# NOAA-GFDL/icebergs

Hardware: AMD Instinct MI355X
Metric: berg_steps_per_sec (higher is better)
Workload: dtype f64; 1 GPU; BASELINE configs[4] per-GPU share with configs[1] physics: 10000000 synthetic bergs/GPU (random mass classes), 360x200 lat-lon ocean grid, RK4 drag+Coriolis+melt+mass spreading, dt=1800 s, ignore_traj=T; bergs_per_gpu=10000000, grid=360x200, exchange=none (1 GPU), bergs_alive_at_end=9999583

## Files before the change

icebergs_amd/csrc/kid_berg_kernel.hpp:

```cpp
#pragma once
#include "kid_device.hpp"
#include "kid_thermo.hpp"
#include "kid_footloose.hpp"
#include "kid_launch_select.hpp"

namespace {
using namespace kid;

struct BergPtrs {
  double *f[KID_NB_F64];
  int32_t *i[KID_NB_I32];
  int64_t *id;
  const double *orient;
};
struct Flags { int has_static, has_fl, store_env, footprint, no_diag; };
typedef __attribute__((address_space(1))) double gdouble;
typedef __attribute__((address_space(1))) int32_t gint32;
typedef __attribute__((address_space(1))) char gchar;
__device__ __forceinline__ double ldg(const double *q, long long k) { return *(const gdouble *)((const gchar *)q + (size_t)((unsigned)k << 3)); }
__device__ __forceinline__ int32_t ldg(const int32_t *q, long long k) { return *(const gint32 *)((const gchar *)q + (size_t)((unsigned)k << 2)); }
__device__ __forceinline__ void keep(double x) { asm volatile("" ::"v"(x)); }
__device__ __forceinline__ void keep(int32_t x) { asm volatile("" ::"v"(x)); }
__device__ __forceinline__ void stg(double *q, long long k, double v) { *(gdouble *)((gchar *)q + (size_t)((unsigned)k << 3)) = v; }
__device__ __forceinline__ void stg(int32_t *q, long long k, int32_t v) { *(gint32 *)((gchar *)q + (size_t)((unsigned)k << 2)) = v; }
template <int K> struct Fl {
#define KID_X(name, k1, k2, k3) static __device__ __forceinline__ int name(const Flags &f) { if constexpr (K == 1) return k1; else if constexpr (K == 2) return k2; else if constexpr (K == 3) return k3; else return f.name; }
  KID_X(has_static, 0, 0, 0) KID_X(has_fl, 0, 1, 0) KID_X(store_env, 0, f.store_env, 1) KID_X(footprint, 0, 0, 0) KID_X(no_diag, 0, 0, 0)
#undef KID_X
};

#ifndef KID_WAVES_PER_EU
#define KID_WAVES_PER_EU 2
#endif
#ifndef KID_HOT_WG
#define KID_HOT_WG 64
#endif
#ifdef KID_EXP_NO_PRIO
#define KID_PRIO_ON false
#else
#define KID_PRIO_ON true
#endif
#ifndef KID_GENERAL_WAVES_PER_EU
#define KID_GENERAL_WAVES_PER_EU 2
#endif
struct StageTab { double *val; int32_t *key; unsigned long long *mask; long long cap; };
enum { KID_RB_NX8 = 10, KID_RB_NX4 = 4 };
struct RebinTab { BergPtrs dst; const void *xs[KID_RB_NX8 + KID_RB_NX4]; void *xd[KID_RB_NX8 + KID_RB_NX4]; int n8, n4; unsigned long long moved, surplus; };
struct Redo { int *list; int *count; long long k0, klen; int *lane; int step;
              int *fl_cursor; int32_t *fl_counter; long long fl_capacity; int fl_iNg; unsigned fl_step;
              StageTab st{};
              const RebinTab *rb = nullptr; const unsigned *perm = nullptr; };
constexpr unsigned long long rb_bit(int f) { return 1ull << f; }
constexpr unsigned long long KID_RB_DYN = rb_bit(KID_B_LON) | rb_bit(KID_B_LAT) | rb_bit(KID_B_UVEL) | rb_bit(KID_B_VVEL) | rb_bit(KID_B_AXN) | rb_bit(KID_B_AYN) |
                                          rb_bit(KID_B_BXN) | rb_bit(KID_B_BYN) | rb_bit(KID_B_XI) | rb_bit(KID_B_YJ);
constexpr unsigned long long KID_RB_ENV = rb_bit(KID_B_UO) | rb_bit(KID_B_VO) | rb_bit(KID_B_UI) | rb_bit(KID_B_VI) | rb_bit(KID_B_UA) | rb_bit(KID_B_VA) |
                                          rb_bit(KID_B_SSH_X) | rb_bit(KID_B_SSH_Y) | rb_bit(KID_B_SST) | rb_bit(KID_B_SSS) | rb_bit(KID_B_CN) | rb_bit(KID_B_HI);
constexpr unsigned long long rb_thermo_fields(int K) {
  return rb_bit(KID_B_MASS) | rb_bit(KID_B_THICKNESS) | rb_bit(KID_B_WIDTH) | rb_bit(KID_B_LENGTH) | rb_bit(KID_B_MASS_OF_BITS) | (K == 3 ? KID_RB_ENV : 0ull);
}
static_assert(KID_NB_F64 <= 64, "one bit per fp64 field");
typedef const __attribute__((address_space(4))) RebinTab cRebinTab;
template <bool REBIN> struct DstTab { static __device__ __forceinline__ const BergPtrs &get(const BergPtrs &b, const Redo &) { return b; } };
template <> struct DstTab<true> { static __device__ __forceinline__ const auto &get(const BergPtrs &, const Redo &r) { return ((cRebinTab *)r.rb)->dst; } };
template <class BD> __device__ __forceinline__ void rebin_copy_row(const BergPtrs &b, const BD &bd, const unsigned *perm, unsigned long long m, bool cell, long long k) {
  const long long ks = (long long)perm[k];
  int32_t ci = 0, cj = 0;
  if (cell) { ci = ldg(b.i[KID_BI_INE], ks); cj = ldg(b.i[KID_BI_JNE], ks); }
  while (m != 0ull) {
    int f[8];
    double v[8];
#pragma unroll
    for (int q = 0; q < 8; ++q) { f[q] = (m != 0ull) ? (int)__ffsll((long long)m) - 1 : -1; m &= m - 1ull; }
#pragma unroll
    for (int q = 0; q < 8; ++q) v[q] = (f[q] >= 0) ? ldg(b.f[f[q]], ks) : 0.;
#pragma unroll
    for (int q = 0; q < 8; ++q) if (f[q] >= 0) stg(bd.f[f[q]], k, v[q]);
  }
  if (cell) { stg(bd.i[KID_BI_INE], k, ci); stg(bd.i[KID_BI_JNE], k, cj); }
}
#ifdef KID_EXP_NUM_VGPR
#define KID_NUM_VGPR_ATTR __attribute__((amdgpu_num_vgpr(KID_EXP_NUM_VGPR)))
#else
#define KID_NUM_VGPR_ATTR
#endif
#ifndef KID_FLP_SLOTS
#define KID_FLP_SLOTS KID_MAXRUN
#define KID_FLP_CHUNK 10
#endif
#ifndef KID_HOT3_SLOTS
#define KID_HOT3_SLOTS 11
#define KID_HOT3_CHUNK 11
#endif
template <bool RK, bool OLD_ORDER, unsigned PH, bool FAST, int K> struct HotCfg {
#if defined(KID_EXACT_MATH) || defined(KID_EXP_NO_HOT3)
  static constexpr bool three = false;
#else
  static constexpr bool three = FAST && RK && OLD_ORDER && (K == 1 || K == 3) && (PH & PH_EVOLVE) != 0 && KID_HOT_WG == 64;
#endif
  static constexpr int slots = three ? KID_HOT3_SLOTS : ((FAST && K == 2) ? KID_FLP_SLOTS : KID_MAXRUN);
  static constexpr int chunk = three ? KID_HOT3_CHUNK : ((FAST && K == 2) ? KID_FLP_CHUNK : KID_CHUNK);
  static constexpr int waves = !FAST ? KID_GENERAL_WAVES_PER_EU : (three ? 3 : KID_WAVES_PER_EU);
};
template <bool S> __device__ __forceinline__ auto &scatter_of(Seg &seg, StageSeg &sseg) { if constexpr (S) return sseg; else return seg; }
template <bool RK, bool OLD_ORDER, unsigned PH, bool FAST, int K = 0, bool STAGE = false, bool REBIN = false>
__global__ void KID_NUM_VGPR_ATTR __launch_bounds__(FAST ? KID_HOT_WG : 256, (HotCfg<RK, OLD_ORDER, PH, FAST, K>::waves)) berg_kernel(const DevGrid *__restrict__ gtab, const kid_params *__restrict__ pp, const BergPtrs *__restrict__ bt, const long long n,
                                                   double *__restrict__ acc, const size_t ncell, const Flags fl, const Redo redo) {
  static_assert(!REBIN || (FAST && RK && OLD_ORDER && !STAGE && (K == 1 || K == 3) && PH == (PH_EVOLVE | PH_THERMO | PH_SPREAD)), "the re-binning instance is a plain hot build");
  const kid_params &p = *pp;
  const BergPtrs &b = *bt;
  const auto &bd = DstTab<REBIN>::get(b, redo);
  const DevGrid &g = *gtab;
  constexpr bool SCATTER = (PH & (PH_THERMO | PH_SPREAD)) != 0;
  constexpr int WG_WAVES = FAST ? KID_HOT_WG / 64 : 4;
  using Cfg = HotCfg<RK, OLD_ORDER, PH, FAST, K>;
  constexpr int SLOTS = Cfg::slots, CHUNK = Cfg::chunk;
  __shared__ double lds_vals[SCATTER ? seg_lds_doubles(WG_WAVES, CHUNK) : 1];
  __shared__ int lds_ints[seg_lds_ints(WG_WAVES, CHUNK)];
  __shared__ __attribute__((aligned(16))) double lds_pk[FAST ? WG_WAVES * SLOTS * PK_STRIDE : 2];
  const long long total = FAST ? redo.klen : (long long)(*redo.count);
  const long long bdim = FAST ? (long long)KID_HOT_WG : (long long)blockDim.x;
  long long tid = (long long)blockIdx.x * bdim + threadIdx.x;
  for (bool first = true; FAST ? first : (tid - threadIdx.x < total); first = false, tid += (long long)gridDim.x * bdim) {
  KID_TICK(-1);
  if (FAST && KID_PRIO_ON) __builtin_amdgcn_s_setprio(3);
  const bool inrange = tid < total;
  const long long k = inrange ? (FAST ? redo.k0 + tid : (long long)redo.list[tid]) : 0ll;
  const long long kk = inrange ? k : (n - 1);
  if constexpr (STAGE) { if (inrange) redo.st.key[k] = -1; }
  long long ks = kk;
  [[maybe_unused]] double x8[KID_RB_NX8];
  [[maybe_unused]] int32_t x4[KID_RB_NX4];
  if constexpr (REBIN) {
    ks = (long long)redo.perm[kk];
    cRebinTab &rb = *(cRebinTab *)redo.rb;
#pragma unroll
    for (int q = 0; q < KID_RB_NX8; ++q) x8[q] = (q < rb.n8) ? ldg((const double *)rb.xs[q], ks) : 0.;
#pragma unroll
    for (int q = 0; q < KID_RB_NX4; ++q) x4[q] = (q < rb.n4) ? ldg((const int32_t *)rb.xs[KID_RB_NX8 + q], ks) : 0;
  }
  const int32_t alive_v = ldg(b.i[KID_BI_ALIVE], ks);
  const int32_t lane_v = FAST ? ldg(redo.lane ? (const int32_t *)redo.lane : (const int32_t *)b.i[KID_BI_ALIVE], ks) : 0;
  BergDyn d;
  d.ine = ldg(b.i[KID_BI_INE], ks); d.jne = ldg(b.i[KID_BI_JNE], ks);
  d.xi = ldg(b.f[KID_B_XI], ks); d.yj = ldg(b.f[KID_B_YJ], ks);
  d.lon = ldg(b.f[KID_B_LON], ks); d.lat = ldg(b.f[KID_B_LAT], ks);
  d.uvel = ldg(b.f[KID_B_UVEL], ks); d.vvel = ldg(b.f[KID_B_VVEL], ks);
  d.uvel_prev = 0.; d.vvel_prev = 0.;
  d.axn = 0.; d.ayn = 0.; d.bxn = 0.; d.byn = 0.;
  if (PH & PH_EVOLVE) {
    d.axn = ldg(b.f[KID_B_AXN], ks); d.ayn = ldg(b.f[KID_B_AYN], ks);
    if (!RK) { d.bxn = ldg(b.f[KID_B_BXN], ks); d.byn = ldg(b.f[KID_B_BYN], ks); }
  }
  BergThermo t;
  t.M = ldg(b.f[KID_B_MASS], ks); t.T = ldg(b.f[KID_B_THICKNESS], ks); t.W = ldg(b.f[KID_B_WIDTH], ks); t.L = ldg(b.f[KID_B_LENGTH], ks);
  t.n_bonds = Sw<K>::iceberg_bonds_on(p) ? ldg(b.i[KID_BI_N_BONDS], ks) : 0;
  t.static_berg = Fl<K>::has_static(fl) ? ldg(b.f[KID_B_STATIC_BERG], ks) : 0.;
  const bool halo = Fl<K>::has_static(fl) ? (ldg(b.f[KID_B_HALO_BERG], ks) >= 0.5) : false;
  constexpr bool SCATTER_ = (PH & (PH_THERMO | PH_SPREAD)) != 0;
  constexpr bool PARK = FAST && SCATTER_ && (PH & PH_EVOLVE) != 0;
  constexpr bool LATE_PARK = PARK && (PH & PH_FL) != 0;
  static_assert(!REBIN || PARK, "the re-binning instance reads its row at the head of the kernel only (ks); the loads further down use kk");
  double park_ms = 0., park_bits = 0., park_hd = 0., park_flk = 0., park_flbits = 0., park_flbergy = 0.;
  if constexpr (PARK) {
    park_ms = ldg(b.f[KID_B_MASS_SCALING], ks); park_bits = ldg(b.f[KID_B_MASS_OF_BITS], ks);
    park_hd = (PH & PH_THERMO) ? ldg(b.f[KID_B_HEAT_DENSITY], ks) : 0.;
    if (Fl<K>::has_fl(fl)) {
      park_flk = ldg(b.f[KID_B_FL_K], ks); park_flbits = ldg(b.f[KID_B_MASS_OF_FL_BITS], ks); park_flbergy = ldg(b.f[KID_B_MASS_OF_FL_BERGY_BITS], ks);
    }
  }
  bool was_alive = inrange && (alive_v != 0);
  if (FAST && redo.lane) { if (was_alive && lane_v >= redo.step) was_alive = false; }
  KID_TICK(11);
  if constexpr (REBIN) {
    cRebinTab &rb = *(cRebinTab *)redo.rb;
    if (inrange) {
#pragma unroll
      for (int q = 0; q < KID_RB_NX8; ++q) if (q < rb.n8) stg((double *)rb.xd[q], kk, x8[q]);
#pragma unroll
      for (int q = 0; q < KID_RB_NX4; ++q) if (q < rb.n4) stg((int32_t *)rb.xd[KID_RB_NX8 + q], kk, x4[q]);
      if (rb.surplus != 0ull) rebin_copy_row(b, bd, redo.perm, rb.surplus, false, kk);
      if (!was_alive) rebin_copy_row(b, bd, redo.perm, rb.moved & (KID_RB_DYN | rb_thermo_fields(K)), true, kk);
    }
  }
  if (__ballot(was_alive) == 0ull) {
    keep(d.ine); keep(d.jne); keep(d.xi); keep(d.yj); keep(d.lon); keep(d.lat); keep(d.uvel); keep(d.vvel); keep(d.axn); keep(d.ayn);
    keep(d.bxn); keep(d.byn); keep(t.M); keep(t.T); keep(t.W); keep(t.L); keep(t.n_bonds); keep(t.static_berg);
    keep(park_ms); keep(park_bits); keep(park_hd); keep(park_flk); keep(park_flbits); keep(park_flbergy);
    continue;
  }
  double *scal = acc - KID_NSCALAR;

  const int mykey = was_alive ? g.idx(d.ine, d.jne) : -1;
  double latref_s = 0., latref_c = 1.;
  if constexpr (FAST && RK && (PH & PH_EVOLVE) != 0) {
    if (grid_latlon<K>(g) && g.latref) { const long long c2 = 2ll * (mykey < 0 ? 0 : mykey); latref_s = ldg(g.latref, c2); latref_c = ldg(g.latref, c2 + 1); }
  }
  Seg seg;
  [[maybe_unused]] StageSeg sseg{};
  if constexpr (!FAST) seg = make_runs(mykey, (lds_double *)lds_vals, (lds_int *)lds_ints, CHUNK);
  const lds_double *pk = nullptr;
  if (FAST) {
    lds_double *wpk = (lds_double *)lds_pk + (threadIdx.x >> 6) * (SLOTS * PK_STRIDE);
    const int lane = (int)__lane_id();
    const gchar *gp = (const gchar *)g.pkt;
    static_assert(PK_SIZE * 8 == 34 * 16 && (PK_STRIDE * 8) % 16 == 0 && (PK_GSTRIDE * 8) % 16 == 0, "packet = 34 lanes x 16 bytes, 16-byte aligned slots");
    int myslot;
    {
    const unsigned loff = (unsigned)lane * 16u;
    unsigned long long rem = __ballot(mykey >= 0);
    int nslot = 0;
    myslot = 0;
    while (rem != 0ull) {
      const int u = (int)__ffsll((long long)rem) - 1;
      const int cu = __builtin_amdgcn_readlane(mykey, u);
      const bool mine = mykey == cu;
      if (mine) myslot = nslot;
      if (nslot < SLOTS && lane < 34)
        __builtin_amdgcn_global_load_lds((const __attribute__((address_space(1))) void *)(gp + (size_t)cu * (size_t)(PK_GSTRIDE * 8) + loff),
                                         (__attribute__((address_space(3))) void *)(wpk + nslot * PK_STRIDE), 16, 0, 0);
      rem &= ~__ballot(mine);
      ++nslot;
    }
    seg = make_runs(mykey, (lds_double *)lds_vals, (lds_int *)lds_ints, CHUNK);
    if (myslot >= SLOTS) {
      if (was_alive) {
        const int slot = atomicAdd(redo.count, 1); redo.list[slot] = (int)kk; if (redo.lane) redo.lane[kk] = redo.step + 1;
        if constexpr (REBIN) rebin_copy_row(b, bd, redo.perm, ((cRebinTab *)redo.rb)->moved & (KID_RB_DYN | rb_thermo_fields(K)), true, kk);
      }
      was_alive = false;
    }
    }
    if (KID_PRIO_ON) __builtin_amdgcn_s_setprio(0);
    KID_TICK(12);
    asm volatile("s_waitcnt vmcnt(0)" ::: "memory");
    __builtin_amdgcn_fence(__ATOMIC_ACQ_REL, "wavefront");
    KID_TICK(13);
    if (__ballot(was_alive) == 0ull) continue;
    pk = wpk + (myslot < SLOTS ? myslot : 0) * PK_STRIDE;
  }
  t.alive = was_alive;
  if constexpr (PARK) {
    lds_double *row = seg.val + (int)__lane_id();
    row[0 * KID_ROW] = t.M; row[1 * KID_ROW] = t.T; row[2 * KID_ROW] = t.W; row[3 * KID_ROW] = t.L;
    row[4 * KID_ROW] = park_ms; row[5 * KID_ROW] = park_bits; row[6 * KID_ROW] = park_hd;
    if (Fl<K>::has_fl(fl)) { row[7 * KID_ROW] = park_flk; row[8 * KID_ROW] = park_flbits; row[9 * KID_ROW] = park_flbergy; }
  }
  Env e = {};
  unsigned tickets = 0u;
  int err = 0;
  bool env_dirty = false;
  bool bail = false;
  bool skipped = false;

  if ((PH & PH_INTERP) || (!OLD_ORDER && (PH & (PH_EVOLVE | PH_THERMO)))) {
    if (PH & PH_INTERP) {
      if (was_alive && !halo) { interp_flds<K>(p, CellOf<FAST>::make(g, pk, d.ine, d.jne), d.xi, d.yj, e); env_dirty = true; }
    } else {
      e.uo = ldg(b.f[KID_B_UO], kk); e.vo = ldg(b.f[KID_B_VO], kk); e.ui = ldg(b.f[KID_B_UI], kk); e.vi = ldg(b.f[KID_B_VI], kk);
      e.ua = ldg(b.f[KID_B_UA], kk); e.va = ldg(b.f[KID_B_VA], kk); e.ssh_x = ldg(b.f[KID_B_SSH_X], kk); e.ssh_y = ldg(b.f[KID_B_SSH_Y], kk);
      e.sst = ldg(b.f[KID_B_SST], kk); e.sss = ldg(b.f[KID_B_SSS], kk); e.cn = ldg(b.f[KID_B_CN], kk); e.hi = ldg(b.f[KID_B_HI], kk); e.od = ldg(b.f[KID_B_OD], kk);
    }
  }

  if (!RK) KID_TICK(2);
  if (PH & PH_EVOLVE) {
    const bool moves = was_alive && (t.static_berg < 0.5);
    if (moves) {
      const BergGeom bg{t.M, t.T, t.W, t.L, t.n_bonds};
      if (RK) {
        if constexpr (!FAST) { if (grid_latlon<K>(g) && g.latref) { const long long c2 = 2ll * g.idx(d.ine, d.jne); latref_s = ldg(g.latref, c2); latref_c = ldg(g.latref, c2 + 1); } }
        rk4_step<OLD_ORDER, FAST, K>(g, p, bg, e, d, tickets, err, bail, pk, latref_s, latref_c);
      }
      else verlet_step<OLD_ORDER, FAST, K>(g, p, bg, e, d, tickets, err, bail, pk);
      if constexpr (PARK) {
        KID_PHASE_FENCE();
        const lds_double *row = seg.val + (int)__lane_id();
        t.M = row[0 * KID_ROW]; t.T = row[1 * KID_ROW]; t.W = row[2 * KID_ROW]; t.L = row[3 * KID_ROW];
        park_ms = row[4 * KID_ROW];
        if constexpr (!LATE_PARK) { park_bits = row[5 * KID_ROW]; park_hd = row[6 * KID_ROW]; }
        if (Fl<K>::has_fl(fl)) { park_flk = row[7 * KID_ROW]; park_flbits = row[8 * KID_ROW]; if constexpr (!LATE_PARK) park_flbergy = row[9 * KID_ROW]; }
      }
      if (FAST && bail) {
        const int slot = atomicAdd(redo.count, 1);
        redo.list[slot] = (int)kk;
        if (redo.lane) redo.lane[kk] = redo.step + 1;
        skipped = true; tickets = 0u; err = 0;
        if constexpr (REBIN) rebin_copy_row(b, bd, redo.perm, ((cRebinTab *)redo.rb)->moved & (KID_RB_DYN | rb_thermo_fields(K)), true, kk);
      } else {
        if (d.ine < g.isc || d.ine > g.iec || d.jne < g.jsc || d.jne > g.jec) {
          bool back = false;
          if constexpr (!FAST) {
            const int nic = g.iec - g.isc + 1;
            const int i2 = d.ine > g.iec ? d.ine - nic : (d.ine < g.isc ? d.ine + nic : d.ine);
            if (p.periodic_reentry && g.Lx > 0. && d.jne >= g.jsc && d.jne <= g.jec && i2 >= g.isc && i2 <= g.iec) {
              const GlbCell cell2{g, g.idx(i2, d.jne)};
              int perr = 0; bool pbail = false;
              double xi2, yj2;
              if (!pos_within_cell<false>(g, p, cell2, d.lon, d.lat, i2, d.jne, xi2, yj2, perr, pbail)) err = 1;
              d.ine = i2; d.xi = xi2; d.yj = yj2;
              stg(bd.f[KID_B_UVEL_OLD], kk, d.uvel); stg(bd.f[KID_B_VVEL_OLD], kk, d.vvel); stg(bd.f[KID_B_LON_OLD], kk, d.lon); stg(bd.f[KID_B_LAT_OLD], kk, d.lat);
              back = true;
            }
          }
          if (!back) t.alive = false;
        }
        stg(bd.f[KID_B_LON], kk, d.lon); stg(bd.f[KID_B_LAT], kk, d.lat); stg(bd.f[KID_B_UVEL], kk, d.uvel); stg(bd.f[KID_B_VVEL], kk, d.vvel);
        stg(bd.f[KID_B_AXN], kk, d.axn); stg(bd.f[KID_B_AYN], kk, d.ayn); stg(bd.f[KID_B_BXN], kk, d.bxn); stg(bd.f[KID_B_BYN], kk, d.byn);
        stg(bd.f[KID_B_XI], kk, d.xi); stg(bd.f[KID_B_YJ], kk, d.yj);
        stg(bd.i[KID_BI_INE], kk, d.ine); stg(bd.i[KID_BI_JNE], kk, d.jne);
        if (!RK) { stg(bd.f[KID_B_UVEL_PREV], kk, d.uvel_prev); stg(bd.f[KID_B_VVEL_PREV], kk, d.vvel_prev); }
      }
    }
    const unsigned long long bt = __ballot(tickets != 0u);
    if (bt) {
      double ts = wave_sum((double)tickets);
      if (__lane_id() == 0) unsafeAtomicAdd(scal + KID_S_NSPEEDING_TICKETS, ts);
    }
  }
  KID_PHASE_FENCE();
  KID_MARK("evolve_done"); KID_TICK(6);

  if (PH & PH_FL) {
    if (was_alive && !skipped && t.alive) {
      const FlChildCtx cx{redo.fl_cursor, redo.fl_counter, n, redo.fl_capacity, redo.fl_iNg, redo.fl_step};
      if constexpr (PARK) {
        bool touched = false;
        footloose_core(g, p, b, cx, kk, d.ine, d.jne, CellOf<FAST>::make(g, pk, d.ine, d.jne).area(), park_ms, t.static_berg, t.M, t.T, t.W, t.L, park_flk, park_flbits, touched, acc, ncell, scal);
        if (touched) {
          park_flbits = ldg(b.f[KID_B_MASS_OF_FL_BITS], kk); park_flbergy = ldg(b.f[KID_B_MASS_OF_FL_BERGY_BITS], kk);
          if constexpr (LATE_PARK) seg.val[(int)__lane_id() + 9 * KID_ROW] = park_flbergy;
        }
      } else {
        footloose_one(g, p, b, cx, kk, acc, ncell, scal);
        t.M = ldg(b.f[KID_B_MASS], kk); t.T = ldg(b.f[KID_B_THICKNESS], kk); t.W = ldg(b.f[KID_B_WIDTH], kk); t.L = ldg(b.f[KID_B_LENGTH], kk);
      }
    }
  }

  if (PH & (PH_THERMO | PH_SPREAD)) {
    const bool active = t.alive && !skipped;
    if constexpr (STAGE) { sseg.val = redo.st.val; sseg.cap = redo.st.cap; sseg.row = kk; sseg.mask = 0ull; }
    auto &sg = scatter_of<STAGE>(seg, sseg);
    if (!FAST) seg = make_runs(active ? g.idx(d.ine, d.jne) : -1, (lds_double *)lds_vals, (lds_int *)lds_ints);
    const typename CellOf<FAST>::type cellv = CellOf<FAST>::make(g, pk, d.ine, d.jne);
    constexpr bool HOTCHECKED = FAST && (PH & PH_EVOLVE) != 0 && K != 0;
    if constexpr (LATE_PARK) {
      const lds_double *row = seg.val + (int)__lane_id();
      park_bits = row[5 * KID_ROW]; park_hd = row[6 * KID_ROW];
      if (Fl<K>::has_fl(fl)) park_flbergy = row[9 * KID_ROW];
    }
    if constexpr (PARK) { t.mass_scaling = park_ms; t.mass_of_bits = park_bits; t.heat_density = park_hd; }
    else {
      t.mass_scaling = ldg(b.f[KID_B_MASS_SCALING], kk);
      t.mass_of_bits = ldg(b.f[KID_B_MASS_OF_BITS], kk);
      t.heat_density = (PH & PH_THERMO) ? ldg(b.f[KID_B_HEAT_DENSITY], kk) : 0.;
    }
    if (PARK && Fl<K>::has_fl(fl)) { t.mass_of_fl_bits = park_flbits; t.mass_of_fl_bergy_bits = park_flbergy; t.fl_k = park_flk; }
    else if (Fl<K>::has_fl(fl)) {
      t.mass_of_fl_bits = ldg(b.f[KID_B_MASS_OF_FL_BITS], kk); t.mass_of_fl_bergy_bits = ldg(b.f[KID_B_MASS_OF_FL_BERGY_BITS], kk);
      t.fl_k = ldg(b.f[KID_B_FL_K], kk);
    } else { t.mass_of_fl_bits = 0.; t.mass_of_fl_bergy_bits = 0.; t.fl_k = 0.; }
    t.start_mass = (Sw<K>::diag_mask(p) & KID_DIAG_MELT_BY_CLASS) ? ldg(b.f[KID_B_START_MASS], kk) : 0.;
    t.start_year = 0; t.start_day = 0.;
    if (PH & PH_THERMO) {
      if (!OLD_ORDER && (PH & PH_EVOLVE) && (PH & PH_INTERP)) {
        if (active) { interp_flds<K, HOTCHECKED>(p, cellv, d.xi, d.yj, e); env_dirty = true; }
      }
      if (OLD_ORDER || (!Sw<K>::mts(p) && !Sw<K>::dem(p) && halo)) {
        const double od_keep = e.od;
        if (active) { interp_flds<K, HOTCHECKED>(p, cellv, d.xi, d.yj, e); env_dirty = true; }
        if (PH & PH_INTERP) e.od = od_keep;
      }
      if (env_dirty && Fl<K>::store_env(fl) && was_alive && !skipped) {
        stg(bd.f[KID_B_UO], kk, e.uo); stg(bd.f[KID_B_VO], kk, e.vo); stg(bd.f[KID_B_UI], kk, e.ui); stg(bd.f[KID_B_VI], kk, e.vi);
        stg(bd.f[KID_B_UA], kk, e.ua); stg(bd.f[KID_B_VA], kk, e.va); stg(bd.f[KID_B_SSH_X], kk, e.ssh_x); stg(bd.f[KID_B_SSH_Y], kk, e.ssh_y);
        stg(bd.f[KID_B_SST], kk, e.sst); stg(bd.f[KID_B_SSS], kk, e.sss); stg(bd.f[KID_B_CN], kk, e.cn); stg(bd.f[KID_B_HI], kk, e.hi);
        if (PH & PH_INTERP) stg(bd.f[KID_B_OD], kk, e.od);
        env_dirty = false;
      }
      KID_PHASE_FENCE();
      KID_MARK("thermo_interp_done"); KID_TICK(7);
      const BergThermo before = t;
      if constexpr ((PH & PH_TSPREAD) != 0) {
        const TSpreadArgs ts{d.xi, d.yj, b.orient ? b.orient[kk] : p.initial_orientation, Fl<K>::footprint(fl) != 0};
        thermodynamics<true, K>(g, p, cellv, t, e, d.uvel, d.vvel, d.lat, d.ine, d.jne, active, acc, ncell, sg, scal, &ts);
      } else thermodynamics<false, K>(g, p, cellv, t, e, d.uvel, d.vvel, d.lat, d.ine, d.jne, active, acc, ncell, sg, scal);
      if (active) {
        stg(bd.f[KID_B_MASS], kk, t.M); stg(bd.f[KID_B_THICKNESS], kk, t.T); stg(bd.f[KID_B_WIDTH], kk, t.W); stg(bd.f[KID_B_LENGTH], kk, t.L);
        if (REBIN || t.mass_of_bits != before.mass_of_bits) stg(bd.f[KID_B_MASS_OF_BITS], kk, t.mass_of_bits);
        if (Fl<K>::has_fl(fl)) {
          stg(bd.f[KID_B_MASS_OF_FL_BITS], kk, t.mass_of_fl_bits); stg(bd.f[KID_B_MASS_OF_FL_BERGY_BITS], kk, t.mass_of_fl_bergy_bits);
          stg(bd.f[KID_B_FL_K], kk, t.fl_k);
          if (t.mass_scaling != before.mass_scaling) {
            stg(bd.f[KID_B_MASS_SCALING], kk, t.mass_scaling);
            stg(bd.i[KID_BI_START_YEAR], kk, t.start_year); stg(bd.f[KID_B_START_DAY], kk, t.start_day);
          }
        }
      }
      if constexpr (REBIN) {
        if (was_alive && !skipped && !active) rebin_copy_row(b, bd, redo.perm, ((cRebinTab *)redo.rb)->moved & rb_thermo_fields(K), false, kk);
      }
      KID_PHASE_FENCE();
      KID_MARK("thermo_done"); KID_TICK(8);
    }
    if (PH & PH_SPREAD) {
      const bool act2 = t.alive && !skipped;
      if ((Sw<K>::add_weight_to_ocean(p) && !Sw<K>::time_average_weight(p)) || Sw<K>::find_melt_using_spread_mass(p))
        spread_mass<K>(g, p, cellv, t, d.uvel, d.vvel, d.ine, d.jne, d.xi, d.yj, act2, acc, ncell, sg, Fl<K>::footprint(fl) != 0,
                       (K == 0 && b.orient) ? b.orient[kk] : p.initial_orientation);
      if (!Fl<K>::no_diag(fl)) berg_diagnostics<K>(g, p, cellv, t, d.uvel, d.vvel, d.ine, d.jne, act2, acc, ncell, sg);
    }
    if (FAST && KID_PRIO_ON) __builtin_amdgcn_s_setprio(3);
    if constexpr (STAGE) { if (inrange && active) { redo.st.key[kk] = g.idx(d.ine, d.jne); redo.st.mask[kk] = sseg.mask; } }
    else seg_flush(seg, acc, ncell);
    KID_MARK("spread_done"); KID_TICK(9);
  }

  if (was_alive && !skipped) {
    if (!t.alive) stg(bd.i[KID_BI_ALIVE], kk, 0);
    if (env_dirty && Fl<K>::store_env(fl)) {
      stg(bd.f[KID_B_UO], kk, e.uo); stg(bd.f[KID_B_VO], kk, e.vo); stg(bd.f[KID_B_UI], kk, e.ui); stg(bd.f[KID_B_VI], kk, e.vi);
      stg(bd.f[KID_B_UA], kk, e.ua); stg(bd.f[KID_B_VA], kk, e.va); stg(bd.f[KID_B_SSH_X], kk, e.ssh_x); stg(bd.f[KID_B_SSH_Y], kk, e.ssh_y);
      stg(bd.f[KID_B_SST], kk, e.sst); stg(bd.f[KID_B_SSS], kk, e.sss); stg(bd.f[KID_B_CN], kk, e.cn); stg(bd.f[KID_B_HI], kk, e.hi);
      if (PH & PH_INTERP) stg(bd.f[KID_B_OD], kk, e.od);
    }
  }
  const unsigned long long be = __ballot(err != 0);
  if (be && __lane_id() == 0) unsafeAtomicAdd(scal + KID_S_ERROR_COUNT, (double)__popcll(be));
  KID_TICK(10); KID_TICK(99);
  }
}

}
```

icebergs_amd/csrc/kid_thermo.hpp:

```cpp
#pragma once
#include "kid_device.hpp"

namespace kid {

#ifndef KID_EXP_MAXRUN
#define KID_EXP_MAXRUN 16
#endif
#ifndef KID_EXP_CHUNK
#define KID_EXP_CHUNK 12
#endif
constexpr int KID_MAXRUN = KID_EXP_MAXRUN;
constexpr int KID_CHUNK = KID_EXP_CHUNK;
constexpr int KID_ROW = 66;
struct Seg {
  lds_double *val;
  lds_int *head;
  lds_int *len;
  lds_int *cell;
  lds_int *plane;
  unsigned long long heads;
  int R;
  int npend;
  int chunk;
  static constexpr bool stage = false;
};
constexpr int seg_lds_doubles(int waves, int chunk = KID_CHUNK) { return waves * chunk * KID_ROW + 4; }
constexpr int seg_lds_ints(int waves, int chunk = KID_CHUNK) { return waves * (3 * 64 + chunk); }

__device__ __forceinline__ double wave_sum(double v) {
#pragma unroll
  for (int d = 32; d >= 1; d >>= 1) v += __shfl_xor(v, d);
  return v;
}
__device__ __forceinline__ Seg make_runs(int key, lds_double *vals, lds_int *ints, int chunk = KID_CHUNK) {
  Seg s;
  const int lane = (int)__lane_id(), wave = (int)(threadIdx.x >> 6);
  s.chunk = chunk;
  s.val = vals + wave * (chunk * KID_ROW);
  lds_int *base = ints + wave * (3 * 64 + chunk);
  s.head = base; s.len = base + 64; s.cell = base + 128; s.plane = base + 192;
  const int prev = __shfl_up(key, 1);
  const bool is_head = (lane == 0) || (prev != key);
  const unsigned long long heads = __ballot(is_head);
  s.heads = heads;
  s.R = __popcll(heads);
  if (is_head) {
    const int r = __popcll(heads & ((1ull << lane) - 1ull));
    const unsigned long long above = (lane == 63) ? 0ull : (heads >> (lane + 1));
    const int next = above ? lane + 1 + (int)__ffsll((long long)above) - 1 : 64;
    s.head[r] = lane; s.len[r] = next - lane; s.cell[r] = key;
  }
  s.npend = 0;
  __builtin_amdgcn_wave_barrier();
  return s;
}
__device__ __noinline__ void seg_flush_impl(lds_double *val, lds_int *head, lds_int *len, lds_int *cell, lds_int *plane,
                                            int R, int npend, double *acc, size_t ncell) {
  __builtin_amdgcn_fence(__ATOMIC_ACQ_REL, "wavefront");
  const int lane = (int)__lane_id();
  const float rR = __builtin_amdgcn_rcpf((float)R);
  const int nitems = npend * R;
  const int P = (nitems * 4 <= 64) ? 4 : ((nitems * 2 <= 64) ? 2 : 1);
  const int lg = (P == 4) ? 2 : ((P == 2) ? 1 : 0);
  for (int base = 0; base < nitems; base += (64 >> lg)) {
    const int item = base + (lane >> lg), part = lane & (P - 1);
    const bool live = item < nitems;
    const int it = live ? item : 0;
    int q = (int)((float)it * rR), r = it - q * R;
    if (r < 0) { q -= 1; r += R; } else if (r >= R) { q += 1; r -= R; }
    const int h = head[r], n = len[r], c = cell[r];
    const int per = (n + P - 1) >> lg;
    const int t0 = part * per, t1 = (t0 + per < n) ? t0 + per : n;
    double sum = 0.;
    const lds_double *v = val + q * KID_ROW + h;
    int t = t0;
    for (; t + 4 <= t1; t += 4) {
      const double a0 = v[t], a1 = v[t + 1], a2 = v[t + 2], a3 = v[t + 3];
      sum += a0; sum += a1; sum += a2; sum += a3;
    }
    if (t < t1) {
      const double a0 = v[t], a1 = v[t + 1], a2 = v[t + 2];
      sum += a0;
      if (t + 1 < t1) sum += a1;
      if (t + 2 < t1) sum += a2;
    }
    if (P >= 2) {
      const double s1 = __shfl_down(sum, 1);
      if (P == 2) sum = sum + s1;
      else {
        const double s2 = __shfl_down(sum, 2), s3 = __shfl_down(sum, 3);
        sum = ((sum + s1) + s2) + s3;
      }
    }
    if (live && part == 0 && c >= 0 && sum != 0.) unsafeAtomicAdd(acc + (size_t)plane[q] * ncell + (size_t)c, sum);
  }
  __builtin_amdgcn_fence(__ATOMIC_ACQ_REL, "wavefront");
}
__device__ __forceinline__ void seg_flush(Seg &s, double *acc, size_t ncell) {
  if (s.npend > 0) seg_flush_impl(s.val, s.head, s.len, s.cell, s.plane, s.R, s.npend, acc, ncell);
  s.npend = 0;
}
__device__ __forceinline__ void cell_add(double *acc, size_t ncell, int plane, int c, double v, Seg &s, bool active) {
  (void)c;
#ifdef KID_EXP_NO_ATOMICS
  if (active && v == 1.2345e-300) acc[(size_t)plane * ncell + c] = v;
  return;
#endif
  s.val[s.npend * KID_ROW + (int)__lane_id()] = active ? v : 0.0;
  s.plane[s.npend] = plane;
  s.npend += 1;
  if (s.npend == s.chunk) seg_flush(s, acc, ncell);
}

enum : int {
  KID_ST_W = KID_A_MASS_ON_OCEAN,
  KID_ST_VAR = KID_ST_W + 9,
  KID_ST_IFU = KID_ST_VAR + 4,
  KID_ST_HEAT = KID_ST_IFU + 1,
  KID_ST_CORE = KID_ST_HEAT + 1,
  KID_ST_N = KID_ST_CORE + (KID_NACC - KID_NACC_CORE)
};
static_assert(KID_ST_N <= 64, "one mask bit per staging slot");
__host__ __device__ constexpr int stage_slot(int plane) { return plane < KID_A_MASS_ON_OCEAN ? plane : plane - KID_NACC_CORE + KID_ST_CORE; }
__device__ __forceinline__ double on_ocean_term(double w, double var, double Ifu) { return w * var * Ifu; }
struct StageSeg {
  double *val;
  long long cap, row;
  unsigned long long mask;
  static constexpr bool stage = true;
  __device__ __forceinline__ void put(int slot, double v) { val[(size_t)slot * (size_t)cap + (size_t)row] = v; mask |= 1ull << slot; }
};
__device__ __forceinline__ void cell_add(double *, size_t, int plane, int, double v, StageSeg &s, bool active) {
  if (active) s.put(stage_slot(plane), v);
}
__device__ __forceinline__ void seg_flush(StageSeg &, double *, size_t) {}

__device__ __noinline__ double kid_pow(double x, double y) { return pow(x, y); }
#ifdef KID_EXACT_MATH
__device__ __forceinline__ double kid_powr(double x, double y) { return kid_pow(x, y); }
#else
__device__ __noinline__ double kid_powr(double x, double y) { return (x == 0.) ? 0. : exp(y * log(x)); }
#endif
#ifdef KID_EXACT_MATH
__device__ __forceinline__ double kid_mul_rpow5(double a, double x) { return a / kid_pow(x, 0.2); }
__device__ __forceinline__ double kid_pow08(double x) { return kid_pow(x, 0.8); }
#else
__device__ __noinline__ double kid_rpow5_slow(double x) { return 1. / kid_powr(x, 0.2); }
__device__ __forceinline__ bool kid_rpow5_fast_range(double x) { return x > 1e-30 && x < 1e30; }
__device__ __forceinline__ double kid_rpow5_newton(double x) {
  double r = (double)__builtin_amdgcn_exp2f(-0.2f * __builtin_amdgcn_logf((float)x));
#pragma unroll
  for (int it = 0; it < 2; ++it) {
    const double r2 = r * r, r4 = r2 * r2;
    const double e = __builtin_fma(-x, r4 * r, 1.0);
    r = __builtin_fma(r, 0.2 * e, r);
  }
  return r;
}
__device__ __forceinline__ double kid_mul_rpow5(double a, double x) {
  return a * (__builtin_expect(kid_rpow5_fast_range(x), 1) ? kid_rpow5_newton(x) : kid_rpow5_slow(x));
}
__device__ __forceinline__ double kid_pow08(double x) {
  return __builtin_expect(kid_rpow5_fast_range(x), 1) ? x * kid_rpow5_newton(x) : kid_powr(x, 0.8);
}
#endif

struct BergThermo {
  double M, T, W, L, mass_scaling, mass_of_bits, mass_of_fl_bits, mass_of_fl_bergy_bits, fl_k, heat_density;
  double start_mass, start_day, static_berg;
  int start_year, n_bonds;
  bool alive;
};

__device__ __forceinline__ int minloc_abs10(const double *tab, double v) {
  int k = 0; double best = fabs(tab[0] - v);
#pragma unroll
  for (int q = 1; q < 10; ++q) { const double d = fabs(tab[q] - v); if (d < best) { best = d; k = q; } }
  return k;
}

template <int K = 0, class CELL, class SEG>
__device__ __forceinline__ void spread_mass(const DevGrid &g, const kid_params &p, const CELL &cellv, const BergThermo &b, double uvel, double vvel,
                                            int i, int j, double x, double y, bool active, double *acc, size_t ncell, SEG &seg, bool footprint, double theta);
struct TSpreadArgs { double xi, yj, theta; bool footprint; };
template <bool TSPREAD = false, int K = 0, class CELL, class SEG>
__device__ __forceinline__ void thermodynamics(const DevGrid &g, const kid_params &p, const CELL &cellv, BergThermo &b, const Env &e,
                                               double uvel, double vvel, double lat, int i, int j, bool active,
                                               double *acc, size_t ncell, SEG &seg, double *scal, const TSpreadArgs *ts = nullptr) {
  constexpr double perday = 1. / 86400.;
  const double dt = p.dt;
  const Rcp rdt = kid_rcp(dt);
  const int c = g.idx(i, j);
  const double SST = e.sst;
  double SSS = e.sss;
  const double IC = dmin(1., e.cn + p.sicn_shift);
  const double M = b.M, T = b.T, W = b.W, L = b.L;
  const double Vol = T * W * L;
  const Rcp rVol = kid_rcp(Vol);
  double du = uvel - e.uo, dv = vvel - e.vo;
  const double dvo = kid_sqrt_nn(kid_fma(du, du, dv * dv));
  du = e.ua - e.uo; dv = e.va - e.vo;
  const double dva = kid_sqrt_nn(kid_fma(du, du, dv * dv));
#ifdef KID_EXACT_MATH
  const double Ss = 1.5 * kid_pow(dva, 0.5) + 0.1 * dva;
#else
  const double Ss = kid_fma(1.5, kid_sqrt_nn(dva), 0.1 * dva);
#endif
  const double dvo08 = kid_pow08(dvo);
  double Mv = dmax(kid_fma(7.62e-3, SST, 1.29e-3 * (SST * SST)), 0.) * perday;
  double Mb = dmax(kid_mul_rpow5(0.58 * dvo08 * (SST + 4.0), L), 0.) * perday;
  const double cos_ic = (__ballot(IC != 0.) == 0ull) ? 1.0 : cos(p.pi * (IC * IC * IC));
  double Me = dmax(1. / 12. * (SST + 2.) * Ss * (1 + cos_ic), 0.) * perday;
  const bool has_fl = b.mass_of_fl_bits > 0.;
  const double Mv_fl = Mv, Me_fl = Me;
  const double N_max = Sw<K>::hexagonal_icebergs(p) ? 6.0 : 4.0;
  double N_bonds = 0.;
  if (Sw<K>::use_mixed_melting(p) || Sw<K>::allow_bergs_to_roll(p)) {
    if (Sw<K>::iceberg_bonds_on(p)) N_bonds = (double)b.n_bonds;
    if (b.static_berg == 1) N_bonds = N_max;
  }
  if (Sw<K>::melt_icebergs_as_ice_shelf(p) || Sw<K>::use_mixed_melting(p)) {
    if (!p.use_mixed_layer_salinity_for_thermo) SSS = 35.0;
    double Ms = dmax(find_basal_melt(g, p, dvo, lat, SSS, SST, p.Use_three_equation_model != 0, T), 0.);
    if ((p.melt_cutoff >= 0.) && p.apply_thickness_cutoff_to_bergs_melt) {
      const double Dn = (p.rho_bergs / RHO_SEAWATER) * T;
      if ((g.ocean_depth[c] - Dn) < p.melt_cutoff) Ms = 0.;
    }
    if (Sw<K>::use_mixed_melting(p)) {
      Me = ((N_max - N_bonds) / N_max) * (Mv + Me);
      Mv = 0.0;
      Mb = (((N_max - N_bonds) / N_max) * (Mb)) + (N_bonds / N_max) * Ms;
    } else { Mv = 0.0; Me = 0.0; Mb = Ms; }
  }
  if (Sw<K>::set_melt_rates_to_zero(p)) { Mv = 0.0; Mb = 0.0; Me = 0.0; }
  double Tn, nVol, Mnew, dMb, dMv, dMe, dM, Ln1 = 0., Wn1 = 0., Ln, Wn;
  if (Sw<K>::use_operator_splitting(p)) {
    Tn = dmax(kid_fma(-Mb, dt, T), 0.);
    nVol = Tn * W * L; const double Mnew1 = (nVol * rVol) * M; dMb = M - Mnew1;
    Ln1 = dmax(kid_fma(-Mv, dt, L), 0.); Wn1 = dmax(kid_fma(-Mv, dt, W), 0.);
    nVol = Tn * Wn1 * Ln1; const double Mnew2 = (nVol * rVol) * M; dMv = Mnew1 - Mnew2;
    Ln = dmax(kid_fma(-Me, dt, Ln1), 0.); Wn = dmax(kid_fma(-Me, dt, Wn1), 0.);
    nVol = Tn * Wn * Ln; Mnew = (nVol * rVol) * M; dMe = Mnew2 - Mnew;
    dM = M - Mnew;
  } else {
    Ln = dmax(kid_fma(-(Mv + Me), dt, L), 0.); Wn = dmax(kid_fma(-(Mv + Me), dt, W), 0.); Tn = dmax(kid_fma(-Mb, dt, T), 0.);
    nVol = Tn * Wn * Ln; Mnew = (nVol * rVol) * M; dM = M - Mnew;
    dMb = (M * rVol) * (W * L) * Mb * dt;
    dMe = (M * rVol) * (T * (W + L)) * Me * dt;
    dMv = (M * rVol) * (T * (W + L)) * Mv * dt;
  }
  double fl_k = b.fl_k;
  if (Sw<K>::footloose(p) && fl_k >= 0) {
    const double l_c = p.pi / (2. * sqrt(2.));
    const double l_b3 = 3. * l_c * kid_root4(FL_LW_C * p.fl_youngs * FL_B_C1 * kid_cube(Tn));
    if (L > l_b3) {
      const double fb = Tn * (1. - p.rho_bergs / RHO_SEAWATER), kd = Tn - fb;
      if (W > l_b3) fl_k = fl_k + (dMe / fb - dMv / kd) / p.rho_bergs;
      else {
        const double dMv_l = dMv * (Wn1 + W) / (2. * (Ln1 + W));
        const double dMe_l = dMe * (Wn + Wn1) / (2. * (Ln + Wn1));
        fl_k = fl_k + (dMe_l / fb - dMv_l / kd) / p.rho_bergs;
      }
      if (fl_k < 0) fl_k = 0;
    }
  }
  double Lfl = 0, Wfl = 0, Tfl = 0, Tnfl = 0, Lnfl = 0, Wnfl = 0, Mnew_fl, dMfl = 0., dMb_fl = 0., dMv_fl = 0., dMe_fl = 0.;
  if (has_fl) {
    fl_bits_dimensions_inl<K>(p, T, Lfl, Wfl, Tfl);
    const double Mfl = b.mass_of_fl_bits, Volfl = Lfl * Wfl * Tfl;
    const double Mb_fl = dmax(kid_mul_rpow5(0.58 * dvo08 * (SST + 4.0), Lfl), 0.) * perday;
    Tnfl = dmax(Tfl - Mb_fl * dt, 0.);
    if (Sw<K>::use_operator_splitting(p)) {
      double nVolfl = Tnfl * Wfl * Lfl; const double Mnew1_fl = (nVolfl / Volfl) * Mfl; dMb_fl = Mfl - Mnew1_fl;
      Lnfl = dmax(Lfl - Mv_fl * dt, 0.); Wnfl = dmax(Wfl - Mv_fl * dt, 0.);
      nVolfl = Tnfl * Wnfl * Lnfl; const double Mnew2_fl = (nVolfl / Volfl) * Mfl; dMv_fl = Mnew1_fl - Mnew2_fl;
      Lnfl = dmax(Lnfl - Me_fl * dt, 0.); Wnfl = dmax(Wnfl - Me_fl * dt, 0.);
      nVolfl = Tnfl * Wnfl * Lnfl; Mnew_fl = (nVolfl / Volfl) * Mfl; dMe_fl = Mnew2_fl - Mnew_fl;
    } else {
      Lnfl = dmax(Lfl - (Mv_fl + Me_fl) * dt, 0.); Wnfl = dmax(Wfl - (Mv_fl + Me_fl) * dt, 0.);
      const double nVolfl = Tnfl * Wnfl * Lnfl; Mnew_fl = (nVolfl / Volfl) * Mfl;
      dMb_fl = (Mfl / Volfl) * (Wfl * Lfl) * Mb_fl * dt;
      dMe_fl = (Mfl / Volfl) * (Tfl * (Wfl + Lfl)) * Me_fl * dt;
      dMv_fl = (Mfl / Volfl) * (Tfl * (Wfl + Lfl)) * Mv_fl * dt;
    }
    dMfl = Mfl - Mnew_fl;
  } else Mnew_fl = b.mass_of_fl_bits;
  double dMbitsE = 0., dMbitsM = 0., nMbits = b.mass_of_bits, dMbitsE_fl = 0., dMbitsM_fl = 0., nMbits_fl = b.mass_of_fl_bergy_bits;
  if (Sw<K>::bergy_bit_erosion_fraction(p) > 0.) {
    const double bbef = Sw<K>::bergy_bit_erosion_fraction(p);
    const double Mbits = b.mass_of_bits;
    dMbitsE = bbef * dMe;
    nMbits = Mbits + dMbitsE;
    const double Lbits = dmin(dmin(dmin(L, W), T), 40.);
    const double Abits = (Mbits / p.rho_bergs) / Lbits;
    double Mbb = dmax(kid_mul_rpow5(0.58 * dvo08 * (SST + 2.0), Lbits), 0.) * perday;
    Mbb = p.rho_bergs * Abits * Mbb;
    dMbitsM = dmin(Mbb * dt, nMbits);
    nMbits = nMbits - dMbitsM;
    if (Mnew == 0.) { dMbitsM = dMbitsM + nMbits; nMbits = 0.; }
    if (has_fl) {
      const double Mbits_fl = b.mass_of_fl_bergy_bits;
      dMbitsE_fl = bbef * dMe_fl;
      nMbits_fl = Mbits_fl + dMbitsE_fl;
      const double Lbits_fl = dmin(dmin(dmin(Lfl, Wfl), Tfl), 40.);
      const double Abits_fl = (Mbits_fl / p.rho_bergs) / Lbits_fl;
      double Mbb_fl = dmax(kid_mul_rpow5(0.58 * dvo08 * (SST + 2.0), Lbits_fl), 0.) * perday;
      Mbb_fl = p.rho_bergs * Abits_fl * Mbb_fl;
      dMbitsM_fl = dmin(Mbb_fl * dt, nMbits_fl);
      nMbits_fl = nMbits_fl - dMbitsM_fl;
      if (Mnew_fl == 0.) { dMbitsM_fl = dMbitsM_fl + nMbits_fl; nMbits_fl = 0.; }
    } else { dMbitsE_fl = 0.; dMbitsM_fl = 0.; nMbits_fl = 0.; }
  }
  const double area = cellv.area(), ms = b.mass_scaling;
  const Rcp rarea = kid_rcp(area);
  const bool ok = active && (area != 0.);
  const int dm = Sw<K>::diag_mask(p);
#define KID_ACC(F, v) cell_add(acc, ncell, (F), c, (v), seg, ok)
  double melt = (dM - (dMbitsE - dMbitsM) + dMfl - (dMbitsE_fl - dMbitsM_fl)) * rdt;
  KID_ACC(KID_A_FLOATING_MELT, melt * rarea * ms);
  if (dm & KID_DIAG_MELT_BY_CLASS) {
    const int kc = (lat < 0.) ? minloc_abs10(p.initial_mass_s, b.start_mass) : minloc_abs10(p.initial_mass_n, b.start_mass);
    for (int q = 0; q < 10; ++q) KID_ACC(KID_A_MELT_BY_CLASS + q, (kc == q) ? melt * rarea * ms : 0.);
  }
  melt = melt * b.heat_density;
  {
    const double hv = ok ? melt * ms * dt : 0.;
    if (__ballot(hv != 0.) != 0ull) {
      KID_ACC(KID_A_CALVING_HFLX, melt * rarea * ms);
      if constexpr (SEG::stage) { if (ok) seg.put(KID_ST_HEAT, hv); }
      else {
        const double h = wave_sum(hv);
        if (__lane_id() == 0 && h != 0.) unsafeAtomicAdd(scal + KID_S_NET_HEAT_TO_OCEAN, h);
      }
    }
  }
  melt = dM * rdt; KID_ACC(KID_A_BERG_MELT, melt * rarea * ms);
  if (Sw<K>::bergy_bit_erosion_fraction(p) > 0.) {
    melt = (dMbitsE + dMbitsE_fl) * rdt; KID_ACC(KID_A_BERGY_SRC, melt * rarea * ms);
    melt = (dMbitsM + dMbitsM_fl) * rdt; KID_ACC(KID_A_BERGY_MELT, melt * rarea * ms);
  }
  if (__ballot(has_fl && ok) != 0ull) { melt = dMfl * rdt; KID_ACC(KID_A_FL_BITS_MELT, melt * rarea * ms); }
  if (dm & (KID_DIAG_FL_PARENT_MELT | KID_DIAG_FL_CHILD_MELT | KID_DIAG_MELT_BUOY | KID_DIAG_MELT_EROS | KID_DIAG_MELT_CONV |
            KID_DIAG_MELT_BUOY_FL | KID_DIAG_MELT_EROS_FL | KID_DIAG_MELT_CONV_FL)) {
    const bool parent = fl_k >= 0;
    if (dm & KID_DIAG_FL_PARENT_MELT) KID_ACC(KID_A_FL_PARENT_MELT, parent ? ((dM - (dMbitsE - dMbitsM)) * rdt) * rarea * ms : 0.);
    if (dm & KID_DIAG_FL_CHILD_MELT)
      KID_ACC(KID_A_FL_CHILD_MELT, (parent ? ((dMfl - (dMbitsE_fl - dMbitsM_fl)) * rdt) : ((dM - (dMbitsE - dMbitsM)) * rdt)) * rarea * ms);
    if (dm & KID_DIAG_MELT_BUOY) KID_ACC(KID_A_MELT_BUOY, parent ? (dMb * rdt) * rarea * ms : 0.);
    if (dm & KID_DIAG_MELT_EROS) KID_ACC(KID_A_MELT_EROS, parent ? (dMe * rdt) * rarea * ms : 0.);
    if (dm & KID_DIAG_MELT_CONV) KID_ACC(KID_A_MELT_CONV, parent ? (dMv * rdt) * rarea * ms : 0.);
    const bool flp = parent && (dMfl > 0);
    if (dm & KID_DIAG_MELT_BUOY_FL) KID_ACC(KID_A_MELT_BUOY_FL, parent ? (flp ? (dMb_fl * rdt) * rarea * ms : 0.) : (dMb * rdt) * rarea * ms);
    if (dm & KID_DIAG_MELT_EROS_FL) KID_ACC(KID_A_MELT_EROS_FL, parent ? (flp ? (dMe_fl * rdt) * rarea * ms : 0.) : (dMe * rdt) * rarea * ms);
    if (dm & KID_DIAG_MELT_CONV_FL) KID_ACC(KID_A_MELT_CONV_FL, parent ? (flp ? (dMv_fl * rdt) * rarea * ms : 0.) : (dMv * rdt) * rarea * ms);
  }
  unsigned nerr = (active && area == 0.) ? 1u : 0u;
  if (Sw<K>::allow_bergs_to_roll(p) && N_bonds == 0.) rolling<K>(p, Tn, Wn, Ln);
  if (Sw<K>::Iceberg_melt_without_decay(p)) {
    if constexpr (TSPREAD) {
      BergThermo nb = b;
      nb.mass_of_fl_bits = Mnew_fl; nb.mass_of_fl_bergy_bits = nMbits_fl;
      if (Mnew > 0.) { nb.M = Mnew; nb.mass_of_bits = nMbits; nb.L = Ln; nb.W = Wn; nb.T = Tn; }
      else {
        const double M_edit = Lnfl * Wnfl * Tnfl * p.rho_bergs;
        nb.M = M_edit; nb.mass_of_bits = nMbits; nb.mass_scaling = Mnew_fl * ms / M_edit; nb.L = Lnfl; nb.W = Wnfl; nb.T = Tnfl;
        nb.mass_of_fl_bits = 0.; nb.mass_of_fl_bergy_bits = 0.;
      }
      spread_mass<K>(g, p, cellv, nb, uvel, vvel, i, j, ts->xi, ts->yj, active && (Mnew > 0. || Mnew_fl > 0.), acc, ncell, seg, ts->footprint, ts->theta);
    }
    Mnew = M;
    b.fl_k = fl_k;
  } else {
    b.M = Mnew; b.mass_of_bits = nMbits; b.mass_of_fl_bits = Mnew_fl; b.mass_of_fl_bergy_bits = nMbits_fl;
    b.T = Tn; b.W = dmin(Wn, Ln); b.L = dmax(Wn, Ln); b.fl_k = fl_k;
  }
  unsigned melted = 0u, calved = 0u;
  double fl_src = 0.;
  if (active && Mnew <= 0.) {
    if (Mnew_fl > 0) {
      calved = 1u;
      const double mass = Lnfl * Wnfl * Tnfl * p.rho_bergs;
      b.M = mass; b.L = Lnfl; b.W = Wnfl; b.T = Tnfl;
      nMbits_fl = nMbits_fl * ms;
      b.mass_scaling = Mnew_fl * ms / mass;
      b.mass_of_bits = nMbits_fl / b.mass_scaling;
      b.mass_of_fl_bits = 0.; b.mass_of_fl_bergy_bits = 0.; b.fl_k = -1.;
      b.start_year = p.current_year; b.start_day = p.current_yearday;
      if (area != 0.) fl_src = -(mass * b.mass_scaling / (dt * area));
    } else b.alive = false;
    melted = 1u;
  }
  if (__ballot(fl_src != 0.) != 0ull) KID_ACC(KID_A_FL_BITS_SRC, fl_src);
#undef KID_ACC
  const unsigned long long bm = __ballot(melted != 0u), bc = __ballot(calved != 0u), be = __ballot(nerr != 0u);
  if (__lane_id() == 0) {
    if (bm) unsafeAtomicAdd(scal + KID_S_NBERGS_MELTED, (double)__popcll(bm));
    if (bc) unsafeAtomicAdd(scal + KID_S_NBERGS_CALVED_FL, (double)__popcll(bc));
    if (be) unsafeAtomicAdd(scal + KID_S_ERROR_COUNT, (double)__popcll(be));
  }
}

__device__ __forceinline__ double tri_area(double Ax, double Ay, double Bx, double By, double Cx, double Cy) {
  return fabs(0.5 * ((Ax * (By - Cy)) + (Bx * (Cy - Ay)) + (Cx * (Ay - By))));
}
__device__ __forceinline__ bool in_interval(double Ax, double Ay, double Bx, double By, double px, double py) {
  return (px <= dmax(Ax, Bx)) && (px >= dmin(Ax, Bx)) && (py <= dmax(Ay, By)) && (py >= dmin(Ay, By));
}
__device__ __forceinline__ bool on_line(double Ax, double Ay, double Bx, double By, double qx, double qy) {
  return fabs((qx - Ax) * (By - Ay) - (qy - Ay) * (Bx - Ax)) <= 0.0;
}
__device__ __forceinline__ bool point_in_triangle(double Ax, double Ay, double Bx, double By, double Cx, double Cy, double qx, double qy) {
// ... 217 lines not shown
```

Baseline: 11.38 billion berg-steps/s.

## Group deposit segments by cell from packet-gather loop instead of adjacent-lane runs

The packet-gather loop already visits each distinct cell key per wave, so it now records, for each lane, its slot, the head and length of its cell group and a rank within that group. Segment tables are built from this per-cell grouping rather than from runs of equal adjacent keys. Each lane writes its deposit value to its rank position, so all bergs sharing a cell land in one contiguous run even when they are not adjacent lanes. This cuts the number of runs per wave and the atomic flushes to the grid, at the cost of a little extra ballot and mbcnt work in the loop. Dead lanes are ranked after all live groups, and lanes whose slot is at or beyond SLOTS get a cell of -1 in the table.

```diff
diff --git a/icebergs_amd/csrc/kid_berg_kernel.hpp b/icebergs_amd/csrc/kid_berg_kernel.hpp
--- a/icebergs_amd/csrc/kid_berg_kernel.hpp
+++ b/icebergs_amd/csrc/kid_berg_kernel.hpp
@@ -207,21 +207,28 @@
     int myslot;
     {
     const unsigned loff = (unsigned)lane * 16u;
-    unsigned long long rem = __ballot(mykey >= 0);
-    int nslot = 0;
+    const unsigned long long dead = __ballot(mykey < 0);
+    unsigned long long rem = ~dead;
+    int nslot = 0, base = 0;
+    int myhead = 0, mylen = 0, myrank = 0;
     myslot = 0;
     while (rem != 0ull) {
       const int u = (int)__ffsll((long long)rem) - 1;
       const int cu = __builtin_amdgcn_readlane(mykey, u);
       const bool mine = mykey == cu;
-      if (mine) myslot = nslot;
+      const unsigned long long bm = __ballot(mine);
+      const int cnt = __popcll(bm);
+      if (mine) { myslot = nslot; myhead = base; mylen = cnt; myrank = base + (int)__builtin_amdgcn_mbcnt_hi((unsigned)(bm >> 32), __builtin_amdgcn_mbcnt_lo((unsigned)bm, 0u)); }
       if (nslot < SLOTS && lane < 34)
         __builtin_amdgcn_global_load_lds((const __attribute__((address_space(1))) void *)(gp + (size_t)cu * (size_t)(PK_GSTRIDE * 8) + loff),
                                          (__attribute__((address_space(3))) void *)(wpk + nslot * PK_STRIDE), 16, 0, 0);
-      rem &= ~__ballot(mine);
+      rem &= ~bm;
+      base += cnt;
       ++nslot;
     }
-    seg = make_runs(mykey, (lds_double *)lds_vals, (lds_int *)lds_ints, CHUNK);
+    if (mykey < 0) myrank = base + (int)__builtin_amdgcn_mbcnt_hi((unsigned)(dead >> 32), __builtin_amdgcn_mbcnt_lo((unsigned)dead, 0u));
+    seg = seg_tables((lds_double *)lds_vals, (lds_int *)lds_ints, CHUNK);
+    seg_by_cell(seg, mykey >= 0 && myrank == myhead, myslot, myhead, mylen, myslot < SLOTS ? mykey : -1, nslot, myrank);
     if (myslot >= SLOTS) {
       if (was_alive) {
         const int slot = atomicAdd(redo.count, 1); redo.list[slot] = (int)kk; if (redo.lane) redo.lane[kk] = redo.step + 1;
diff --git a/icebergs_amd/csrc/kid_thermo.hpp b/icebergs_amd/csrc/kid_thermo.hpp
--- a/icebergs_amd/csrc/kid_thermo.hpp
+++ b/icebergs_amd/csrc/kid_thermo.hpp
@@ -18,10 +18,10 @@
   lds_int *len;
   lds_int *cell;
   lds_int *plane;
-  unsigned long long heads;
   int R;
   int npend;
   int chunk;
+  int rank;
   static constexpr bool stage = false;
 };
 constexpr int seg_lds_doubles(int waves, int chunk = KID_CHUNK) { return waves * chunk * KID_ROW + 4; }
@@ -32,17 +32,27 @@
   for (int d = 32; d >= 1; d >>= 1) v += __shfl_xor(v, d);
   return v;
 }
-__device__ __forceinline__ Seg make_runs(int key, lds_double *vals, lds_int *ints, int chunk = KID_CHUNK) {
+__device__ __forceinline__ Seg seg_tables(lds_double *vals, lds_int *ints, int chunk = KID_CHUNK) {
   Seg s;
-  const int lane = (int)__lane_id(), wave = (int)(threadIdx.x >> 6);
+  const int wave = (int)(threadIdx.x >> 6);
   s.chunk = chunk;
   s.val = vals + wave * (chunk * KID_ROW);
   lds_int *base = ints + wave * (3 * 64 + chunk);
   s.head = base; s.len = base + 64; s.cell = base + 128; s.plane = base + 192;
+  s.R = 0; s.npend = 0; s.rank = (int)__lane_id();
+  return s;
+}
+__device__ __forceinline__ void seg_by_cell(Seg &s, bool first, int slot, int head, int len, int cell, int ncells, int rank) {
+  if (first) { s.head[slot] = head; s.len[slot] = len; s.cell[slot] = cell; }
+  s.R = ncells; s.rank = rank;
+  __builtin_amdgcn_wave_barrier();
+}
+__device__ __forceinline__ Seg make_runs(int key, lds_double *vals, lds_int *ints, int chunk = KID_CHUNK) {
+  Seg s = seg_tables(vals, ints, chunk);
+  const int lane = (int)__lane_id();
   const int prev = __shfl_up(key, 1);
   const bool is_head = (lane == 0) || (prev != key);
   const unsigned long long heads = __ballot(is_head);
-  s.heads = heads;
   s.R = __popcll(heads);
   if (is_head) {
     const int r = __popcll(heads & ((1ull << lane) - 1ull));
@@ -106,7 +116,7 @@
   if (active && v == 1.2345e-300) acc[(size_t)plane * ncell + c] = v;
   return;
 #endif
-  s.val[s.npend * KID_ROW + (int)__lane_id()] = active ? v : 0.0;
+  s.val[s.npend * KID_ROW + s.rank] = active ? v : 0.0;
   s.plane[s.npend] = plane;
   s.npend += 1;
   if (s.npend == s.chunk) seg_flush(s, acc, ncell);
```

After: 11.68 billion berg-steps/s (median of 6 runs). +2.7%, better.
